# jank324/lynx

Measured on AMD Instinct MI355X. Metric: particle-element-steps/sec (whole node) + achieved HBM GB/s, Segment.track ParticleBeam, higher is better.
Workload: dtype f32

## Files before the change

### lynx_amd/csrc/lynx_device.hpp

```cpp
#pragma once

#include <hip/hip_runtime.h>

#include <type_traits>

#include "lynx_maps.hpp"
#include "lynx_unit_record.hpp"

namespace lynx {

typedef float lynx_f32x4 __attribute__((ext_vector_type(4)));
typedef double lynx_f64x2 __attribute__((ext_vector_type(2)));
template <typename T, bool VEC> struct VecOf { using type = T; static constexpr int width = 1; };
template <> struct VecOf<float, true> { using type = lynx_f32x4; static constexpr int width = 4; };
template <> struct VecOf<double, true> { using type = lynx_f64x2; static constexpr int width = 2; };

struct LatticeDev {
  const lynx_elem* elems;
  const lynx_step* steps;
  const int32_t* elem_step;
  const void* pool;
  int64_t batch;
  int32_t n_elems;
  int32_t n_steps;
};

template <int BYTES>
struct InlinePool {
  uint4 q[BYTES / 16];
};
constexpr int kInlinePoolSmall = 256, kInlinePoolLarge = 1024;
__device__ __forceinline__ LatticeDev inline_pool_view(const LatticeDev& lat) {
  LatticeDev v = lat;
  v.pool = (const void*)__builtin_amdgcn_kernarg_segment_ptr();
  return v;
}

__device__ __forceinline__ bool steps_pair_up(const lynx_step& run, const lynx_step& cav) {
  return run.kind == LYNX_STEP_RUN && cav.kind == LYNX_STEP_CAVITY && !(run.flags & LYNX_STEP_FLAG_OBSERVE);
}

__device__ __forceinline__ int step_descriptor(const LatticeDev& lat, int s, int merge_pairs) {
  const lynx_step st = lat.steps[s];
  int d = (st.flags & 0xffff) | (st.kind << LYNX_DESC_KIND_SHIFT);
  if (merge_pairs && s + 1 < lat.n_steps && steps_pair_up(st, lat.steps[s + 1])) d |= LYNX_DESC_PAIR;
  return d;
}

constexpr double kEntryConditionLimit = 4.0;
template <typename T>
__device__ __forceinline__ bool cavity_entry_inverse(T c44, T c45, T c54, T c55, T (&ci)[4]) {
  const double a = (double)c44 * (double)c55, b = (double)c45 * (double)c54;
  const double det = a - b;
  ci[0] = (T)((double)c55 / det);
  ci[1] = (T)(-(double)c45 / det);
  ci[2] = (T)(-(double)c54 / det);
  ci[3] = (T)((double)c44 / det);
  return !(fabs(det) * kEntryConditionLimit >= fabs(a) + fabs(b)) || det == 0.0;
}

constexpr int kBuildChunk = 64;
constexpr int kTrackThreads = 256;
constexpr int kPartialStride = 36;

template <typename T> __device__ __forceinline__ T shfl_t(T v, int src) { return __shfl(v, src, 64); }

__host__ __device__ inline int build_chunk(int n_elems, int limit = kBuildChunk) {
  return n_elems < limit ? (n_elems > 1 ? n_elems : 1) : limit;
}
__host__ __device__ inline size_t build_scratch_bytes(int chunk, size_t elem_size) {
  size_t b = (size_t)(chunk + (chunk / 2 + 1) + (chunk / 4 + 1) + 2) * 49 * sizeof(double);
  if (elem_size == 4) b += (size_t)chunk * 49 * sizeof(float);
  return (b + 15) / 16 * 16;
}

struct BuildLds {
  size_t steps;
  size_t energies, tail, end;
  size_t total;
};
__host__ __device__ inline BuildLds build_lds_layout(int chunk, size_t n_steps, size_t elem_size, size_t tail_scalars) {
  BuildLds l{};
  l.steps = build_scratch_bytes(chunk, elem_size);
  l.energies = n_steps * LYNX_STEP_STRIDE;
  l.tail = n_steps + 1;
  l.end = tail_scalars;
  l.total = l.steps + (l.energies + l.tail + l.end) * elem_size;
  return l;
// ... 906 lines not shown
}

template <typename T>
__device__ __forceinline__ void build_to_table(const LatticeDev& lat, const T* __restrict__ energy_in,
                                               T* __restrict__ steps_out, T* __restrict__ energy_out,
                                               int chunk, int merge_pairs) {
  extern __shared__ __attribute__((aligned(16))) unsigned char smem_raw[];
  const BuildLds lds = build_lds_layout(chunk, (size_t)lat.n_steps, sizeof(T), 0);
  T* s_steps = reinterpret_cast<T*>(smem_raw + lds.steps);
  T* s_energy = s_steps + lds.energies;
  const int64_t b = blockIdx.x;
  for (int i = threadIdx.x; i < lat.n_steps * LYNX_STEP_STRIDE; i += blockDim.x) s_steps[i] = T(0);
  __syncthreads();
  build_compose_sample<T>(lat, b, energy_in[b], s_steps, s_energy, smem_raw, chunk);
  table_sinphi<T>(lat, s_steps);
  if (merge_pairs) {
    for (int s = 1; s < lat.n_steps; ++s) {
      if (!steps_pair_up(lat.steps[s - 1], lat.steps[s])) continue;
      T* run = s_steps + (s - 1) * LYNX_STEP_STRIDE;
      T* cav = s_steps + s * LYNX_STEP_STRIDE;
      T v = T(0);
      if (threadIdx.x < 49) {
        const int i = threadIdx.x / 7, j = threadIdx.x - i * 7;
        double acc = (double)cav[i * 7] * (double)run[j];
#pragma unroll
        for (int k = 1; k < 7; ++k) acc = fma((double)cav[i * 7 + k], (double)run[k * 7 + j], acc);
        v = (T)acc;
      }
      T ci[4] = {T(0), T(0), T(0), T(0)};
      bool ill = false;
      if (threadIdx.x == 49) ill = cavity_entry_inverse<T>(cav[4 * 7 + 4], cav[4 * 7 + 5], cav[5 * 7 + 4], cav[5 * 7 + 5], ci);
      __syncthreads();
      if (threadIdx.x < 49) cav[threadIdx.x] = v;
      if (threadIdx.x == 49) {
#pragma unroll
        for (int q = 0; q < 4; ++q) cav[LYNX_ENTRY_OFFSET + q] = ci[q];
        cav[LYNX_FLAGS_OFFSET] = ill ? T(1) : T(0);
      }
      if (threadIdx.x >= 64 && threadIdx.x < 78) run[threadIdx.x - 64] = run[28 + (threadIdx.x - 64)];
      __syncthreads();
    }
  }
  for (int s = threadIdx.x; s < lat.n_steps; s += blockDim.x) {
    const bool ill = s_steps[s * LYNX_STEP_STRIDE + LYNX_FLAGS_OFFSET] != T(0);
    s_steps[s * LYNX_STEP_STRIDE + LYNX_FLAGS_OFFSET] = (T)(step_descriptor(lat, s, merge_pairs) | (ill ? LYNX_DESC_ILL : 0));
  }
  if (lat.n_steps > 0 && threadIdx.x == 0)
    s_steps[(lat.n_steps - 1) * LYNX_STEP_STRIDE + LYNX_ENERGY_OFFSET] = s_energy[lat.n_steps];
  __syncthreads();
  T* dst = steps_out + b * (int64_t)lat.n_steps * LYNX_STEP_STRIDE;
  for (int i = threadIdx.x; i < lat.n_steps * LYNX_STEP_STRIDE; i += blockDim.x) dst[i] = s_steps[i];
  if (energy_out && threadIdx.x == 0) energy_out[b] = s_energy[lat.n_steps];
}

template <typename T>
__global__ __launch_bounds__(256) void k_build(LatticeDev lat, const T* __restrict__ energy_in,
                                                T* __restrict__ steps_out, T* __restrict__ energy_out,
                                                int chunk, int merge_pairs) {
  build_to_table<T>(lat, energy_in, steps_out, energy_out, chunk, merge_pairs);
}

template <typename T, int BYTES>
__global__ __launch_bounds__(256) void k_build_inline(InlinePool<BYTES> , LatticeDev lat,
                                                       const T* __restrict__ energy_in, T* __restrict__ steps_out,
                                                       T* __restrict__ energy_out, int chunk, int merge_pairs) {
  build_to_table<T>(inline_pool_view(lat), energy_in, steps_out, energy_out, chunk, merge_pairs);
}


struct TrackArgs {
  int64_t n_particles;
  int32_t chunks;
  int32_t tiles_per_wg;
  int32_t store;
  int32_t lds_scratch_bytes;
  int64_t in_stride;
  int32_t merged_pairs;
  int32_t n_observers;
  uint32_t tail_seq;
  int32_t tail_wg;
  unsigned int* tail_flag;
  int32_t stash_offset;
  int32_t reversed;
};

__device__ __forceinline__ void announce_tail(const TrackArgs& a) {
  if (a.tail_flag && blockIdx.x == (unsigned)a.tail_wg && threadIdx.x == 0)
    __hip_atomic_store(a.tail_flag, a.tail_seq, __ATOMIC_RELAXED, __HIP_MEMORY_SCOPE_SYSTEM);
}

__device__ __forceinline__ float uniform_value(float v) {
  return __int_as_float(__builtin_amdgcn_readfirstlane(__float_as_int(v)));
}
__device__ __forceinline__ double uniform_value(double v) { return v; }
__device__ __forceinline__ float wave_first(float v) { return uniform_value(v); }
__device__ __forceinline__ double wave_first(double v) {
  const long long bits = __double_as_longlong(v);
  const int lo = __builtin_amdgcn_readfirstlane((int)(bits & 0xffffffffll));
  const int hi = __builtin_amdgcn_readfirstlane((int)(bits >> 32));
  return __longlong_as_double(((long long)hi << 32) | (unsigned int)lo);
}

__device__ __forceinline__ double moment_slot_moved(const double* row, const double* c0, int j) {
  if (j == 6 || j >= 28) return row[j];
  const double n = row[35];
  if (j < 6) return row[j] + n * (row[28 + j] - c0[j]);
  int k = j - 7, i = 0, len = 6;
  while (k >= len) { k -= len; --len; ++i; }
  const int jj = i + k;
  const double ei = row[28 + i] - c0[i], ej = row[28 + jj] - c0[jj];
  return row[j] + ei * row[jj] + row[i] * ej + n * ei * ej;
}

template <bool FULL> struct MomentSet {
  static constexpr int N = FULL ? 21 : 8;
  __host__ __device__ static constexpr int row(int k) { return FULL ? tri_row(k) : (k < 6 ? k : (k == 6 ? 0 : 2)); }
  __host__ __device__ static constexpr int col(int k) { return FULL ? tri_col(k) : (k < 6 ? k : (k == 6 ? 1 : 3)); }
  __host__ __device__ static constexpr int slot(int k) { return 7 + tri_index(row(k), col(k)); }
  __host__ __device__ static constexpr int tri_index(int i, int j) { return i * 6 - (i * (i - 1)) / 2 + (j - i); }
  __host__ __device__ static constexpr int tri_row(int k) {
    int i = 0, len = 6;
    while (k >= len) { k -= len; --len; ++i; }
    return i;
  }
  __host__ __device__ static constexpr int tri_col(int k) {
    int i = 0, len = 6;
    while (k >= len) { k -= len; --len; ++i; }
    return i + k;
  }
};

template <typename T, bool FULL> struct MomentAcc {
  using Set = MomentSet<FULL>;
  double d[6], dd[Set::N], one, cnt;
  __device__ __forceinline__ void clear() {
#pragma unroll
    for (int i = 0; i < 6; ++i) d[i] = 0.0;
#pragma unroll
    for (int i = 0; i < Set::N; ++i) dd[i] = 0.0;
    one = 0.0;
    cnt = 0.0;
  }
  template <int K> __device__ __forceinline__ void products(const double (&e)[6]) {
    if constexpr (K < Set::N) {
      constexpr int r = Set::row(K), c = Set::col(K);
      dd[K] = fma(e[r], e[c], dd[K]);
      products<K + 1>(e);
    }
  }
  __device__ __forceinline__ void add(const T (&z)[7], const T (&shift)[6]) {
    double e[6];
#pragma unroll
    for (int i = 0; i < 6; ++i) {
      e[i] = (double)z[i] - (double)shift[i];
      d[i] += e[i];
    }
    one += (double)z[6];
    cnt += 1.0;
    products<0>(e);
  }
};

typedef float lynx_f32x4u __attribute__((ext_vector_type(4), aligned(4)));
typedef float lynx_f32x3u __attribute__((ext_vector_type(3), aligned(4)));
typedef double lynx_f64x2u __attribute__((ext_vector_type(2), aligned(8)));
typedef unsigned int lynx_u32x4 __attribute__((ext_vector_type(4)));
// ... 104 lines not shown
#pragma unroll
    for (int k = 0; k < Set::N; ++k) f_dd[k] = 0.f;
    f_one = 0.f;
  }
  __device__ __forceinline__ void init() {
    if (MOM == 1 || MOM == 2) acc.clear();
    if (MOM == 3) clear_f();
  }
  __device__ __forceinline__ void begin_iteration() {
    if (MOM == 2) clear_f();
  }
  template <int K> __device__ __forceinline__ void products(const float (&e)[6]) {
    if constexpr (K < Set::N) {
      constexpr int r = Set::row(K), c = Set::col(K);
      f_dd[K] = fmaf(e[r], e[c], f_dd[K]);
      products<K + 1>(e);
    }
  }
  __device__ __forceinline__ void add(const T (&z)[7], const T (&shift)[6]) {
    if (MOM == 1) acc.add(z, shift);
    if (MOM == 2 || MOM == 3) {
      float e[6];
#pragma unroll
      for (int k = 0; k < 6; ++k) {
        e[k] = (float)(z[k] - shift[k]);
        f_d[k] += e[k];
      }
      f_one += (float)z[6];
      products<0>(e);
      if (MOM == 2) acc.cnt += 1.0;
      else f_cnt += 1.f;
    }
  }
  __device__ __forceinline__ void end_iteration() {
    if (MOM == 2) {
#pragma unroll
      for (int k = 0; k < 6; ++k) acc.d[k] += (double)f_d[k];
#pragma unroll
      for (int k = 0; k < Set::N; ++k) acc.dd[k] += (double)f_dd[k];
      acc.one += (double)f_one;
    }
  }
  template <typename R> __device__ __forceinline__ void park(R* slab, int lane) const {
    if (MOM == 3) {
#pragma unroll
      for (int i = 0; i < 6; ++i) slab[i * 65 + lane] = (R)f_d[i];
      slab[6 * 65 + lane] = (R)f_one;
#pragma unroll
      for (int i = 0; i < Set::N; ++i) slab[(7 + i) * 65 + lane] = (R)f_dd[i];
      slab[(7 + Set::N) * 65 + lane] = (R)f_cnt;
    } else {
#pragma unroll
      for (int i = 0; i < 6; ++i) slab[i * 65 + lane] = (R)acc.d[i];
      slab[6 * 65 + lane] = (R)acc.one;
#pragma unroll
      for (int i = 0; i < Set::N; ++i) slab[(7 + i) * 65 + lane] = (R)acc.dd[i];
      slab[(7 + Set::N) * 65 + lane] = (R)acc.cnt;
    }
  }
  template <int K> __device__ static __forceinline__ int slot_scan(int r, int sl) {
    if constexpr (K < Set::N) {
      constexpr int slot = Set::slot(K);
      return slot_scan<K + 1>(r, r == 7 + K ? slot : sl);
    } else {
      return sl;
    }
  }
  __device__ static __forceinline__ int slot_of_row(int r) {
    if (r < 7) return r;
    if (r == 7 + Set::N) return 35;
    return slot_scan<0>(r, 0);
  }
};

template <typename T, int MOM, bool FULL>
__device__ __forceinline__ void workgroup_moment_record(const LaneSums<T, MOM, FULL>& sums, const T (&shift)[6],
                                                        unsigned char* s_scratch, double* __restrict__ out) {
  const int tid = threadIdx.x;
  const int wave = tid >> 6, lane = tid & 63;
  {
    using R = typename MomScratch<MOM>::type;
    using Sums = LaneSums<T, MOM, FULL>;
    constexpr int kRows = Sums::kRows;
    __syncthreads();
    R* slab = reinterpret_cast<R*>(s_scratch) + wave * (kRows * 65);
    sums.park(slab, lane);
    __syncthreads();
    double tot = 0.0;
    if (lane < kRows) {
      const R* row = slab + lane * 65;
#pragma unroll 8
      for (int k = 0; k < 64; ++k) tot += (double)row[k];
    }
    __syncthreads();
    double* s_red = reinterpret_cast<double*>(s_scratch);
    if (lane < kPartialStride) s_red[wave * kPartialStride + lane] = 0.0;
    __syncthreads();
    if (lane < kRows) s_red[wave * kPartialStride + Sums::slot_of_row(lane)] = tot;
    if (lane == 0) {
#pragma unroll
      for (int k = 0; k < 6; ++k) s_red[wave * kPartialStride + 28 + k] = (double)shift[k];
      s_red[wave * kPartialStride + 34] = FULL ? 1.0 : 0.0;
    }
    __syncthreads();
    if (tid < kPartialStride) {
      double v;
      if (tid >= 28 && tid < 35) {
        v = s_red[tid];
      } else {
        v = 0.0;
#pragma unroll
        for (int w = 0; w < kTrackThreads / 64; ++w) v += moment_slot_moved(s_red + w * kPartialStride, s_red + 28, tid);
      }
      out[tid] = v;
    }
  }
}

template <typename T, int UNROLL, bool SCALAR_TABLE>
__device__ __forceinline__ void apply_program_lane(const LatticeDev& lat, int S, const T* g_steps, const T* s_steps,
                                                   T (&z)[UNROLL][7],
                                                   double* s_obs = nullptr ,
                                                   const bool (*live)[UNROLL] = nullptr,
                                                   float* stash = nullptr ) {
  constexpr bool kMapInRegs = sizeof(T) == 4;
  constexpr bool kPairs = kMapInRegs && UNROLL % 2 == 0;
  lynx_f32x2 zp[kPairs ? UNROLL / 2 : 1][7];
  if constexpr (kPairs) {
#pragma unroll
    for (int u = 0; u < UNROLL; u += 2)
#pragma unroll
      for (int c = 0; c < 7; ++c) {
        zp[u / 2][c].x = (float)z[u][c];
        zp[u / 2][c].y = (float)z[u + 1][c];
      }
  }
  int n_obs = 0;
  for (int sidx = 0; sidx < S; ++sidx) {
    bool merged = false;
    const T* table = SCALAR_TABLE ? g_steps : s_steps;
    int desc = (int)uniform_value(table[sidx * LYNX_STEP_STRIDE + LYNX_FLAGS_OFFSET]);
    if (s_obs && (desc & LYNX_STEP_FLAG_OBSERVE)) {
#pragma unroll
      for (int u = 0; u < UNROLL; ++u) {
        double x, y;
        if constexpr (kPairs) {
          x = (u & 1) ? (double)zp[u / 2][0].y : (double)zp[u / 2][0].x;
          y = (u & 1) ? (double)zp[u / 2][2].y : (double)zp[u / 2][2].x;
        } else {
          x = (double)z[u][0];
          y = (double)z[u][2];
        }
        if (!live || (*live)[u]) {
          s_obs[(2 * n_obs + 0) * 256] += x;
          s_obs[(2 * n_obs + 1) * 256] += y;
        }
      }
      ++n_obs;
    }
    if constexpr (kPairs && SCALAR_TABLE && UNROLL == 2) {
      if (desc & LYNX_DESC_PAIR) {
        merged = true;
        ++sidx;
        desc = (int)uniform_value(table[sidx * LYNX_STEP_STRIDE + LYNX_FLAGS_OFFSET]);
      }
    }
    const int skind = (desc >> LYNX_DESC_KIND_SHIFT) & 3, sflags = desc & 0xffff;
    if constexpr (kMapInRegs) {
      T m[LYNX_STEP_SCALARS];
      if (SCALAR_TABLE) {
        const T* tab = g_steps + sidx * LYNX_STEP_STRIDE;
#pragma unroll
        for (int q = 0; q < LYNX_STEP_SCALARS; ++q) m[q] = uniform_value(tab[q]);
      } else {
        const T* tab = s_steps + sidx * LYNX_STEP_STRIDE;
#pragma unroll
        for (int q = 0; q < LYNX_STEP_SCALARS; ++q) m[q] = uniform_value(tab[q]);
      }
      if constexpr (kPairs) {
        const bool rows_form = __builtin_expect(merged && (desc & LYNX_DESC_ILL), 0);
        const int entry = !merged ? kEntryOwn : (rows_form ? kEntryStash : kEntryInverse);
#pragma unroll
        for (int h = 0; h < UNROLL / 2; ++h) {
          if (rows_form) {
            lynx_f32x2 s_in = zp[h][0] * uniform_value(g_steps[(sidx - 1) * LYNX_STEP_STRIDE]);
            lynx_f32x2 d_in = zp[h][0] * uniform_value(g_steps[(sidx - 1) * LYNX_STEP_STRIDE + 7]);
#pragma unroll
            for (int j = 1; j < 7; ++j) {
              s_in = pk_fma(zp[h][j], uniform_value(g_steps[(sidx - 1) * LYNX_STEP_STRIDE + j]), s_in);
              d_in = pk_fma(zp[h][j], uniform_value(g_steps[(sidx - 1) * LYNX_STEP_STRIDE + 7 + j]), d_in);
            }
            *reinterpret_cast<lynx_f32x4*>(stash) = lynx_f32x4{s_in.x, s_in.y, d_in.x, d_in.y};
          }
          apply_step_pair(m, skind, sflags, zp[h], entry, lynx_f32x2{0.f, 0.f}, lynx_f32x2{0.f, 0.f}, stash);
        }
      } else {
#pragma unroll
        for (int u = 0; u < UNROLL; ++u) apply_step<T>(m, skind, sflags, z[u]);
      }
    } else {
      const T* tab = s_steps + sidx * LYNX_STEP_STRIDE;
#pragma unroll
      for (int u = 0; u < UNROLL; ++u) apply_step<T>(tab, skind, sflags, z[u]);
    }
  }
  if constexpr (kPairs) {
#pragma unroll
    for (int u = 0; u < UNROLL; u += 2)
#pragma unroll
      for (int c = 0; c < 7; ++c) {
        z[u][c] = (T)zp[u / 2][c].x;
        z[u + 1][c] = (T)zp[u / 2][c].y;
      }
  }
}

template <typename T, int MOM, bool FULL, int UNROLL, bool XPOSE> constexpr int track_waves_per_simd() {
  if (XPOSE) return 3;
  if (sizeof(T) == 4 && UNROLL == 2 && !FULL && (MOM == 0 || MOM == 3)) return 5;
  return 1;
}

struct TrackLds {
  size_t steps, observers, total, stash, stash_bytes;
};
template <typename T>
__host__ __device__ constexpr TrackLds track_lds_layout(size_t scratch_bytes, size_t S, size_t n_observers) {
  TrackLds l{};
  l.steps = scratch_bytes;
  l.observers = (scratch_bytes + (S * (LYNX_STEP_STRIDE + 1) + 1) * sizeof(T) + 7) / 8 * 8;
  l.total = l.observers + 2 * n_observers * 256 * sizeof(double);
  l.stash = (l.total + 15) / 16 * 16;
  l.stash_bytes = (size_t)kTrackThreads * 4 * sizeof(float);
  return l;
}

template <int UNROLL, bool XPOSE>
struct TileGeometry {
  static constexpr int64_t kTile = (int64_t)kTrackThreads * UNROLL;
  static constexpr int64_t kWaveSpan = 64 * UNROLL;
  static constexpr int64_t kLaneStep = XPOSE ? 1 : kTrackThreads;
  int wave, lane, chunk, tiles_per_wg;
  int64_t end;
  int64_t lane_first;
  __device__ __forceinline__ TileGeometry(int tid, int wave_, int lane_, int chunk_, int tiles_per_wg_, int64_t end_)
      : wave(wave_), lane(lane_), chunk(chunk_), tiles_per_wg(tiles_per_wg_), end(end_),
        lane_first(XPOSE ? (int64_t)wave_ * kWaveSpan + (int64_t)lane_ * UNROLL : (int64_t)tid) {}
  __device__ __forceinline__ int64_t tile_of(int it) const { return (int64_t)chunk * tiles_per_wg + it; }
  __device__ __forceinline__ int64_t wave_base(int64_t tile) const { return tile * kTile + (int64_t)wave * kWaveSpan; }
  __device__ __forceinline__ bool wave_whole(int64_t tile) const { return wave_base(tile) + kWaveSpan <= end; }
  __device__ __forceinline__ int64_t first_of(int64_t tile) const { return tile * kTile + lane_first; }
  __device__ __forceinline__ bool past_end(int64_t tile) const { return XPOSE ? (wave_base(tile) >= end) : (first_of(tile) >= end); }
};

template <typename T, int UNROLL>
__device__ __forceinline__ void wave_tile_fetch_if_whole(const TileGeometry<UNROLL, true> g, const T* src, int64_t tile,
                                                         lynx_u32x4 (&v)[7]) {
  if (g.wave_whole(tile)) wave_tile_fetch(src + g.wave_base(tile) * 7, g.lane, v);
}

template <typename T, int N> __device__ __forceinline__ void apply_single_map(const T (&m0)[N], const T* s_steps, T (&z)[7]) {
  if constexpr (sizeof(T) == 4) apply_step<T>(m0, LYNX_STEP_RUN, 0, z);
  else apply_step<T>(s_steps, LYNX_STEP_RUN, 0, z);
}

template <typename T, int MOM, bool FULL, int UNROLL, bool XPOSE>
__global__ __launch_bounds__(kTrackThreads, (track_waves_per_simd<T, MOM, FULL, UNROLL, XPOSE>())) void k_track_direct(
    LatticeDev lat, TrackArgs a, const T* __restrict__ , const T* p_in, T* p_out,
    T* __restrict__ energy_out, const T* __restrict__ steps_in, double* __restrict__ partials,
    double* __restrict__ obs_partials) {
  static_assert(!XPOSE || (UNROLL * 7 * sizeof(T) == 112), "XPOSE: a lane owns 112 bytes");
  extern __shared__ __attribute__((aligned(16))) unsigned char smem_raw[];
  announce_tail(a);
  const TrackLds lds = track_lds_layout<T>(a.lds_scratch_bytes, lat.n_steps, a.n_observers);
  unsigned char* s_scratch = smem_raw;
  T* s_steps = reinterpret_cast<T*>(smem_raw + lds.steps);
  float* stash = reinterpret_cast<float*>(smem_raw + a.stash_offset) + threadIdx.x * 4;
  double* s_obs = reinterpret_cast<double*>(smem_raw + lds.observers) + threadIdx.x;

  const int tid = threadIdx.x;
  const int wave = tid >> 6, lane = tid & 63;
  const unsigned wg = a.reversed ? gridDim.x - 1u - blockIdx.x : blockIdx.x;
  const int64_t b = wg / a.chunks;
  const int chunk = wg % a.chunks;
  const int64_t end = a.n_particles;
  const int S = lat.n_steps;
  using Geometry = TileGeometry<UNROLL, XPOSE>;
  const Geometry g(tid, wave, lane, chunk, a.tiles_per_wg, end);
  unsigned char* s_wave = s_scratch + wave * kWaveTileBytes;

  const T* src = p_in + b * a.in_stride;
  T* dst = p_out + b * end * 7;
  T zn[XPOSE ? 1 : UNROLL][7];
  lynx_u32x4 vn[XPOSE ? 7 : 1];
  if constexpr (XPOSE) {
    wave_tile_fetch_if_whole(g, src, g.tile_of(0), vn);
  } else {
    const int64_t i0 = g.first_of(g.tile_of(0));
#pragma unroll
    for (int u = 0; u < UNROLL; ++u) {
      const int64_t i = i0 + (int64_t)u * Geometry::kLaneStep;
      load_particle(src + (i < end ? i : (i0 < end ? i0 : 0)) * 7, zn[u]);
    }
  }

  const bool one_run = (S == 1) && (lat.steps[0].kind == LYNX_STEP_RUN) && a.n_observers == 0;
  for (int k = 0; k < 2 * a.n_observers; ++k) s_obs[k * 256] = 0.0;
  constexpr bool kMapInRegs = sizeof(T) == 4;
  const T* g_steps = steps_in + b * (int64_t)S * LYNX_STEP_STRIDE;

  if (S > 0) {
    if (!kMapInRegs) load_steps_sample<T>(g_steps, S, s_steps);
    if (energy_out && chunk == 0 && tid == 0) energy_out[b] = g_steps[(S - 1) * LYNX_STEP_STRIDE + LYNX_ENERGY_OFFSET];
  }

  T m0[kMapInRegs ? 49 : 1];
  if (one_run && kMapInRegs) {
#pragma unroll
    for (int i = 0; i < 49; ++i) m0[i] = uniform_value(g_steps[i]);
  }

  LaneSums<T, MOM, FULL> sums;
  sums.init();
  T shift[6];
#pragma unroll
  for (int i = 0; i < 6; ++i) shift[i] = T(0);

  constexpr bool kLdsResident = XPOSE && sizeof(T) == 8;

  for (int it = 0; it < a.tiles_per_wg; ++it) {
    const int64_t tile = g.tile_of(it);
    const int64_t i0 = g.first_of(tile);
    if (g.past_end(tile)) break;
    if (!kMapInRegs) LYNX_FORGET();
    const bool full = XPOSE && g.wave_whole(tile);
    sums.begin_iteration();

    if constexpr (kLdsResident) {
      T* mine =reinterpret_cast<T*>(s_wave) + lane * (UNROLL * 7);
      if (full) {
        lynx_u32x4* l = reinterpret_cast<lynx_u32x4*>(s_wave);
        wave_fence();
#pragma unroll
        for (int k = 0; k < 7; ++k) l[k * 64 + lane] = vn[k];
        wave_fence();
      }
      if (it + 1 < a.tiles_per_wg) wave_tile_fetch_if_whole(g, src, g.tile_of(it + 1), vn);
#pragma unroll 1
      for (int u = 0; u < UNROLL; ++u) {
        const int64_t i = i0 + u;
        T z[1][7];
        if (full) {
#pragma unroll
          for (int c = 0; c < 7; ++c) z[0][c] = mine[u * 7 + c];
        } else {
          load_particle(src + (i < end ? i : end - 1) * 7, z[0]);
        }
        if (one_run) {
          apply_single_map(m0, s_steps, z[0]);
        } else {
          const bool alive[1] = {i < end};
          apply_program_lane<T, 1, false>(lat, S, g_steps, s_steps, z, a.n_observers ? s_obs : nullptr, &alive);
        }
        if (MOM && it == 0 && u == 0) {
#pragma unroll
          for (int k = 0; k < 6; ++k) shift[k] = wave_first(z[0][k]);
        }
        if (i < end) {
          if (MOM) sums.add(z[0], shift);
          if (a.store) {
            if (full) {
#pragma unroll
              for (int c = 0; c < 7; ++c) mine[u * 7 + c] = z[0][c];
            } else {
              store_particle(dst + i * 7, z[0]);
            }
          }
        }
      }
      if (a.store && full) {
        lynx_u32x4 vo[7];
        const lynx_u32x4* l = reinterpret_cast<const lynx_u32x4*>(s_wave);
        wave_fence();
#pragma unroll
        for (int k = 0; k < 7; ++k) vo[k] = l[k * 64 + lane];
        wave_tile_store(dst + g.wave_base(tile) * 7, lane, vo);
      }
    } else {
      T z[UNROLL][7];
      if constexpr (XPOSE) {
        if (full) {
          wave_tile_to_particles<T, UNROLL>(vn, s_wave, lane, z);
        } else {
#pragma unroll
          for (int u = 0; u < UNROLL; ++u) load_particle(src + (i0 + u < end ? i0 + u : end - 1) * 7, z[u]);
        }
        if (it + 1 < a.tiles_per_wg) wave_tile_fetch_if_whole(g, src, g.tile_of(it + 1), vn);
      } else {
#pragma unroll
        for (int u = 0; u < UNROLL; ++u)
#pragma unroll
          for (int c = 0; c < 7; ++c) z[u][c] = zn[u][c];
        if (it + 1 < a.tiles_per_wg) {
          const int64_t j0 = g.first_of(g.tile_of(it + 1));
#pragma unroll
          for (int u = 0; u < UNROLL; ++u) {
            const int64_t j = j0 + (int64_t)u * Geometry::kLaneStep;
            load_particle(src + (j < end ? j : i0) * 7, zn[u]);
          }
        }
      }
      if (!one_run) {
        bool alive[UNROLL];
#pragma unroll
        for (int u = 0; u < UNROLL; ++u) alive[u] = i0 + (int64_t)u * Geometry::kLaneStep < end;
        apply_program_lane<T, UNROLL, kMapInRegs>(lat, S, g_steps, s_steps, z,
                                                  a.n_observers ? s_obs : nullptr, &alive, stash);
      }
#pragma unroll
      for (int u = 0; u < UNROLL; ++u) {
        const int64_t i = i0 + (int64_t)u * Geometry::kLaneStep;
        if (one_run) apply_single_map(m0, s_steps, z[u]);
        if (MOM && it == 0 && u == 0) {
#pragma unroll
          for (int k = 0; k < 6; ++k) shift[k] = wave_first(z[0][k]);
        }
        if (i < end) {
          if (a.store && !(XPOSE && full)) store_particle(dst + i * 7, z[u]);
          if (MOM) sums.add(z[u], shift);
        }
      }
      if constexpr (XPOSE) {
        if (a.store && full) {
          lynx_u32x4 vo[7];
          wave_tile_from_particles<T, UNROLL>(z, s_wave, lane, vo);
          wave_tile_store(dst + g.wave_base(tile) * 7, lane, vo);
        }
      }
    }
    sums.end_iteration();
  }

  if (a.n_observers) {
    __syncthreads();
    if (tid < 2 * a.n_observers) {
      const double* row = s_obs - threadIdx.x + tid * 256;
      double tot = 0.0;
      for (int k = 0; k < 256; ++k) tot += row[k];
      obs_partials[((int64_t)b * a.chunks + chunk) * (2 * LYNX_MAX_OBSERVERS) + tid] = tot;
    }
  }

  if (MOM) workgroup_moment_record<T, MOM, FULL>(sums, shift, s_scratch, partials + ((int64_t)b * a.chunks + chunk) * kPartialStride);
}

constexpr int kReduceStage = 70;
template <int THREADS, int STAGE> constexpr size_t reduce_lds_bytes() {
  return (size_t)(STAGE + THREADS / kPartialStride + 1) * kPartialStride * sizeof(double);
}

__device__ __forceinline__ void write_moment_record(const double* s, double* dst, int tid) {
  const double n = s[35];
  if (tid < 6) {
    dst[tid] = s[28 + tid] + s[tid] / n;
  } else if (tid == 6) {
    dst[6] = s[6] / n;
  } else if (tid < 28) {
    int k = tid - 7, i = 0, row = 6;
    while (k >= row) { k -= row; --row; ++i; }
    const int j = i + k;
    const bool have = (s[34] != 0.0 || i == j || (i == 0 && j == 1) || (i == 2 && j == 3)) &&
                      __builtin_isfinite(s[i]) && __builtin_isfinite(s[j]);
    dst[tid] = have ? (s[tid] - s[i] * s[j] / n) / n : __longlong_as_double(0x7ff8000000000000ll);
  } else if (tid < 34) {
    dst[tid] = 0.0;
  } else if (tid == 34) {
    dst[34] = s[34];
  } else if (tid == 35) {
    dst[35] = n;
  }
}

struct ReduceLds {
  double *rows, *set, *s;
};
template <int THREADS, int STAGE>
// ... 692 lines not shown
```

### lynx_amd/csrc/lynx_hip.hip

```cpp
#include <hip/hip_runtime.h>
#include <hip/hip_ext.h>
#include <rccl/rccl.h>

#include <algorithm>
#include <array>
#include <cstdio>
#include <cstdlib>
#include <cstring>
#include <map>
#include <mutex>
#include <string>
#include <type_traits>
#include <unordered_map>
#include <vector>

#include "lynx_device.hpp"
#include "lynx_grad.hpp"
#include "lynx_units.hpp"
#include "lynx_grad_units.hpp"
#include "lynx_trace.hpp"
#include "lynx_trace_grad.hpp"
#include "lynx_trace_jvp.hpp"
#include "lynx_moment_loss.hpp"

using namespace lynx;

struct Knobs {
  int xpose = -1;
  int unroll = -1;
  int mom = -1;
  int min_tiles_per_wg = -1;
  int async_build = -1;
  int side_reduce = -1;
  int build_host_wait = -1;
  int gather_overlap = -1;
  int lanes_build_min_batch = 256;
  int piece = 8;
  int pair_levels_fused = 1;
  int merge_steps = 1;
  int reduce_ticket = 1;
  int one_round = -1;
  int track_units = 1;
  int unit_pairs = 1;
  int bwd_units = 1;
  int bwd_merge = 1;
  int bwd_pairs = 1;
  int build_in_tail = 1;
  int small_inline = -1;
  int bwd_reuse_table = 1;
  int host_visible_records = 1;
  int alternate_order = 1;
  int inline_pool = 1;
};

static void load_knobs(Knobs* k) {
  *k = Knobs();
  const struct { const char* name; int* value; } table[] = {
      {"LYNX_XPOSE", &k->xpose}, {"LYNX_UNROLL", &k->unroll}, {"LYNX_MOM", &k->mom},
      {"LYNX_MIN_TILES_PER_WG", &k->min_tiles_per_wg}, {"LYNX_ASYNC_BUILD", &k->async_build},
      {"LYNX_SIDE_REDUCE", &k->side_reduce}, {"LYNX_BUILD_HOST_WAIT", &k->build_host_wait},
      {"LYNX_GATHER_OVERLAP", &k->gather_overlap}, {"LYNX_LANES_BUILD_MIN_BATCH", &k->lanes_build_min_batch},
      {"LYNX_PIECE", &k->piece}, {"LYNX_PAIR_LEVELS_FUSED", &k->pair_levels_fused},
      {"LYNX_MERGE_STEPS", &k->merge_steps},
      {"LYNX_REDUCE_TICKET", &k->reduce_ticket}, {"LYNX_TRACK_UNITS", &k->track_units}, {"LYNX_ONE_ROUND", &k->one_round}, {"LYNX_UNIT_PAIRS", &k->unit_pairs}, {"LYNX_BWD_UNITS", &k->bwd_units},
      {"LYNX_BWD_MERGE", &k->bwd_merge}, {"LYNX_BWD_PAIRS", &k->bwd_pairs}, {"LYNX_BUILD_IN_TAIL", &k->build_in_tail},
      {"LYNX_SMALL_INLINE", &k->small_inline}, {"LYNX_INLINE_POOL", &k->inline_pool}, {"LYNX_ALTERNATE_ORDER", &k->alternate_order}, {"LYNX_HOST_VISIBLE_RECORDS", &k->host_visible_records}, {"LYNX_BWD_REUSE_TABLE", &k->bwd_reuse_table}};
  for (const auto& t : table) {
    const char* v = getenv(t.name);
    if (v && *v) *t.value = atoi(v);
  }
}
static inline int knob(int value, int dflt) { return value >= 0 ? value : dflt; }

struct Scratch {
  void* buf = nullptr;
  size_t bytes = 0;
};

struct lynx_ctx {
  Knobs knobs;
  int device = 0;
  hipStream_t stream = nullptr;
  hipStream_t s_build = nullptr;
  static constexpr int kTableSlots = 3;
  hipEvent_t ev_built[kTableSlots] = {};
  struct BuildOrder {
    hipEvent_t ev_streamed_own[kTableSlots] = {}, ev_mark = nullptr;
    hipEvent_t ev_streamed[kTableSlots] = {};
    bool streamed_valid[kTableSlots] = {};
    bool main_dirty = false;
    const void* main_wrote = nullptr;
    const void* slot_wrote[kTableSlots] = {};

    void main_wrote_build_input() { main_dirty = true; }
    hipEvent_t stop_event(int slot) const { return ev_streamed_own[slot]; }
    void streamed(int slot, bool async, hipEvent_t stop, const void* energy_out) {
      if (slot >= 0) {
        ev_streamed[slot] = stop;
        streamed_valid[slot] = async && stop != nullptr;
        if (!async) main_dirty = true;
        slot_wrote[slot] = energy_out;
      }
      if (energy_out) main_wrote = energy_out;
    }
    hipError_t read_until_here(int slot, hipStream_t main) {
      const hipError_t e = hipEventRecord(ev_streamed_own[slot], main);
      if (e != hipSuccess) return e;
      ev_streamed[slot] = ev_streamed_own[slot];
      streamed_valid[slot] = true;
      return hipSuccess;
    }
    hipError_t order_build(hipStream_t bs, hipStream_t main, int slot, const void* energy, unsigned int* tail_flag,
                           uint32_t tail_value) {
      hipError_t e = hipSuccess;
      if (streamed_valid[slot] && (e = hipStreamWaitEvent(bs, ev_streamed[slot], 0)) != hipSuccess) return e;
      if (tail_flag && (e = hipStreamWaitValue32(bs, tail_flag, tail_value, hipStreamWaitValueGte, 0xffffffffu)) != hipSuccess)
        return e;
      if (main_dirty || (main_wrote && main_wrote == energy)) {
        if ((e = hipEventRecord(ev_mark, main)) != hipSuccess || (e = hipStreamWaitEvent(bs, ev_mark, 0)) != hipSuccess) return e;
        main_dirty = false;
        main_wrote = nullptr;
        for (const void*& w : slot_wrote) w = nullptr;
      } else {
        for (int i = 0; i < kTableSlots; ++i)
          if (i != slot && slot_wrote[i] == energy && energy && streamed_valid[i] &&
              (e = hipStreamWaitEvent(bs, ev_streamed[i], 0)) != hipSuccess)
            return e;
      }
      return hipSuccess;
    }
    void forget_stop_events() {
      for (bool& v : streamed_valid) v = false;
    }
  } order;
  unsigned seq = 0;
  bool main_idle = true;
  bool plain_events = false;
  unsigned long_calls = 0;
  struct FwdTable {
    const lynx_lattice* lat = nullptr;
    uint64_t version = 0;
    const void* energy = nullptr;
    int slot = -1;
    int merged = 0;
    bool units = false;
    size_t energy_bytes = 0;
    unsigned seq = 0;
    bool valid = false;
    void written(const void* dst, size_t bytes) {
// ... 1134 lines not shown
  }
  const int chunk = fit_build_chunk<T>(build_shape<T>(ctx, lat, underneath, true), lat, 0);
  const size_t lds = build_lds_layout(chunk, (size_t)lat->n_steps, sizeof(T), 0).total;
  const auto launch = [&](const auto&... pool) -> int {
    const auto kernel = build_kernel<T>(pool...);
    if constexpr (sizeof...(pool) == 0)
      if (const int stale = sync_pool(ctx, lat)) return stale;
    if (const int refused = allow_lds(ctx, kernel, lds)) return refused;
    hipLaunchKernelGGL(kernel, dim3((unsigned)lat->batch), dim3(256), lds, stream, pool..., dev_view(lat), (const T*)d_energy_in,
                       (T*)d_steps_out, (T*)d_energy_out, chunk, merge_pairs);
    HIP_TRY(ctx, hipGetLastError());
    return LYNX_OK;
  };
  if (const int rc = with_pool_form<T>(lat, lat->prog_pool && ctx->knobs.inline_pool, launch)) return rc;
  if constexpr (sizeof(T) == 4)
    if (d_units) return launch_pack_units(ctx, lat, merge_pairs, stream, d_steps_out, d_units, d_extras);
  return LYNX_OK;
}

int lynx_build_compose(lynx_ctx* ctx, lynx_lattice* lat, const void* d_energy_in, void* d_steps_out,
                       void* d_energy_out) {
  LYNX_MAIN_ENTRY(ctx);
  if (!lat || !d_energy_in || !d_steps_out) return fail(ctx, LYNX_ERR_INVALID, "null argument");
  if (lat->batch > 0x7fffffffLL) return fail(ctx, LYNX_ERR_INVALID, "batch too large");
  const size_t es = dtype_size(lat->dtype);
  LYNX_MAIN_WRITES(ctx, kFeedsBuild, {{d_steps_out, (size_t)lat->batch * lat->n_steps * LYNX_STEP_STRIDE * es},
                                      {d_energy_out, (size_t)lat->batch * es}});
  return with_dtype(lat->dtype, [&](auto zero) {
    return launch_build<decltype(zero)>(ctx, lat, ctx->stream, d_energy_in, d_steps_out, d_energy_out);
  });
}


struct TrackPlan {
  hipEvent_t done = nullptr;
  bool full_cov;
  int unroll;
  int mom_mode;
  bool xpose;
  TrackArgs a;
  size_t lds;
  unsigned grid;
};

template <typename T>
static TrackPlan plan_track(lynx_ctx* ctx, const lynx_lattice* lat, int64_t B, int64_t N, int32_t S, bool moments,
                            bool full_cov) {
  TrackPlan p;
  p.full_cov = full_cov;
  constexpr int P = 16 / (int)sizeof(T);
  const int64_t cus = compute_units(ctx);
  const Knobs& kn = ctx->knobs;
  const int64_t target = 512 * cus;
  p.mom_mode = knob(kn.mom, sizeof(T) == 4 ? 2 : 1);
  if (sizeof(T) == 8 || p.mom_mode < 2 || p.mom_mode > 3) p.mom_mode = sizeof(T) == 4 ? 2 : 1;
  p.a.n_particles = N;
  p.a.store = 0;
  p.a.tail_flag = nullptr;
  p.a.tail_seq = 0;
  p.a.tail_wg = 0;
  p.a.stash_offset = 0;
  p.a.reversed = 0;
  const bool single_map = S == 1 && lat && lat->h_steps[0].kind == LYNX_STEP_RUN &&
                          !(lat->h_steps[0].flags & LYNX_STEP_FLAG_OBSERVE);
  p.xpose = knob(kn.xpose, ((sizeof(T) == 8 || (single_map && !full_cov)) && N >= 8 * 64 * P) ? 1 : 0) != 0;
  int u = knob(kn.unroll, p.xpose ? P : (sizeof(T) == 4 ? (S > 1 ? 2 : 4) : 1));
  if (u != 1 && u != 2 && u != 4) u = 2;
  if (sizeof(T) == 8 && u > 2) u = 2;
  while (u > 1 && B * ((N + 256 * u - 1) / (256 * u)) < 4 * cus) u >>= 1;
  if (u != P) p.xpose = false;
  p.unroll = u;
  const int64_t tile = 256 * (int64_t)u;
  const int64_t ntiles = (N + tile - 1) / tile;
  int64_t min_tpw = std::max(1, knob(kn.min_tiles_per_wg, S > 1 ? 16 : 2));
  while (min_tpw > 1 && B * ((ntiles + min_tpw - 1) / min_tpw) < 4 * cus) --min_tpw;
  int64_t chunks = std::max<int64_t>(1, std::min<int64_t>((ntiles + min_tpw - 1) / min_tpw, (target + B - 1) / B));
  {
    const int64_t one_round = 3 * cus;
    const int cap = knob(kn.one_round, (S <= 1 && B * chunks > one_round && B * chunks <= 4 * one_round) ? 3 : 0);
    if (cap > 0) chunks = std::max<int64_t>(1, std::min<int64_t>(chunks, cap * cus / B));
  }
  int64_t tpw = (ntiles + chunks - 1) / chunks;
  chunks = (ntiles + tpw - 1) / tpw;
  p.a.chunks = (int32_t)chunks;
  p.a.tiles_per_wg = (int32_t)tpw;
  if (p.mom_mode == 2 && kn.mom < 0 && tpw * u <= 32) p.mom_mode = 3;
  if (p.mom_mode == 3 && tpw * u > 64) p.mom_mode = 2;
  size_t scratch = 4 * kPartialStride * sizeof(double);
  if (moments)
    scratch = std::max<size_t>(scratch, (size_t)(full_cov ? kMomSlabScalars : kMomSlabScalarsCompact) * (p.mom_mode >= 2 ? 4 : 8));
  if (p.xpose) scratch = std::max<size_t>(scratch, (size_t)(kTrackThreads / 64) * kWaveTileBytes);
  scratch = (scratch + 15) / 16 * 16;
  p.a.lds_scratch_bytes = (int32_t)scratch;
  p.a.n_observers = lat ? lat->n_observers : 0;
  p.lds = track_lds_layout<T>(scratch, (size_t)S, (size_t)p.a.n_observers).total;
  p.grid = (unsigned)(B * chunks);
  return p;
}

template <typename K, typename... Args>
static int launch_streaming(lynx_ctx* ctx, const TrackPlan& p, K kernel, size_t lds, const Args&... args) {
  int rc = allow_lds(ctx, kernel, lds);
  if (rc) return rc;
  hipEvent_t e0 = nullptr, e1 = p.done;
  if (ctx->profiling) {
    HIP_TRY(ctx, hipEventCreateWithFlags(&e0, timing_event_flags(ctx)));
    HIP_TRY(ctx, hipEventCreateWithFlags(&e1, timing_event_flags(ctx)));
  }
  hipExtLaunchKernelGGL(kernel, dim3(p.grid), dim3(kTrackThreads), (std::uint32_t)lds, ctx->stream, e0, e1, 0u, args...);
  HIP_TRY(ctx, hipGetLastError());
  if (ctx->profiling) ctx->prof_events.emplace_back(e0, e1);
  ctx->last_stream_stop = e1;
  return LYNX_OK;
}

struct DirectLaunch {
  lynx_ctx* ctx;
  const TrackPlan& p;
  const LatticeDev& lv;
  const void *d_energy_in, *d_p_in;
  void *d_p_out, *d_energy_out;
  const void* d_steps;
  double *d_partials, *d_obs;
};

template <typename T, int MOM, bool FULL, int UNROLL, bool XPOSE>
static int launch_direct_inst(const DirectLaunch& l) {
  return launch_streaming(l.ctx, l.p, k_track_direct<T, MOM, FULL, UNROLL, XPOSE>, l.p.lds, l.lv, l.p.a, (const T*)l.d_energy_in,
                          (const T*)l.d_p_in, (T*)l.d_p_out, (T*)l.d_energy_out, (const T*)l.d_steps, l.d_partials, l.d_obs);
}

template <typename T, int MOM, bool FULL, int U>
static int launch_direct_mu(const DirectLaunch& l) {
  if constexpr (U * 7 * sizeof(T) == 112) {
    if (l.p.xpose) return launch_direct_inst<T, MOM, FULL, U, true>(l);
  }
  return launch_direct_inst<T, MOM, FULL, U, false>(l);
}

template <typename T, int MOM, bool FULL>
static int launch_direct_m(const DirectLaunch& l) {
  switch (l.p.unroll) {
    case 1: return launch_direct_mu<T, MOM, FULL, 1>(l);
    case 2: return launch_direct_mu<T, MOM, FULL, 2>(l);
    default:
      if constexpr (sizeof(T) == 4) return launch_direct_mu<T, MOM, FULL, 4>(l);
      else return fail(l.ctx, LYNX_ERR_INVALID, "float64: at most 2 particles per lane");
  }
}

template <typename T>
static int launch_direct(const DirectLaunch& l, bool moments) {
  const int mom = moments ? l.p.mom_mode : 0;
  if (mom == 0) return launch_direct_m<T, 0, false>(l);
  if constexpr (sizeof(T) == 4) {
    if (mom == 3) return l.p.full_cov ? launch_direct_m<T, 3, true>(l) : launch_direct_m<T, 3, false>(l);
    return l.p.full_cov ? launch_direct_m<T, 2, true>(l) : launch_direct_m<T, 2, false>(l);
  } else {
    return l.p.full_cov ? launch_direct_m<T, 1, true>(l) : launch_direct_m<T, 1, false>(l);
  }
}


static int proposed_class(const lynx_lattice* lat, int32_t first, int32_t last) {
  int rank = 1;
  for (int32_t e = first; e < last; ++e) {
// ... 2181 lines not shown
```

Before: 13970 billion.

## Add tapered chunk plan and wave-local moment reduction in tracking kernel

Adds a launch plan in which the last chunks of each sample handle a single tile each, with chunk-major workgroup ordering, so the tail of the grid finishes more evenly. This mode is gated behind a new LYNX_TAPER knob that defaults to off. The moment record reduction is also rewritten to run inside each wave, using 16-row passes with shuffles and wave fences in place of several workgroup barriers. Each wave's record is kept inside its own slab, which cuts synchronisation in the epilogue but depends on the slab size assertions holding.

```diff
diff --git a/lynx_amd/csrc/lynx_device.hpp b/lynx_amd/csrc/lynx_device.hpp
--- a/lynx_amd/csrc/lynx_device.hpp
+++ b/lynx_amd/csrc/lynx_device.hpp
@@ -4,6 +4,7 @@
 
 #include <type_traits>
 
+#include "lynx_launch_plan.hpp"
 #include "lynx_maps.hpp"
 #include "lynx_unit_record.hpp"
 
@@ -1076,6 +1077,9 @@
   unsigned int* tail_flag;
   int32_t stash_offset;
   int32_t reversed;
+  TilePlan tiles;
+  int32_t chunk_major;
+  int32_t batch;
 };
 
 __device__ __forceinline__ void announce_tail(const TrackArgs& a) {
@@ -1346,35 +1350,49 @@
     using R = typename MomScratch<MOM>::type;
     using Sums = LaneSums<T, MOM, FULL>;
     constexpr int kRows = Sums::kRows;
+    constexpr int kSlabBytes = kRows * 65 * (int)sizeof(R);
+    static_assert(kRows <= 32, "two passes of 16 rows");
+    static_assert(kPartialStride * 8 + 7 <= kSlabBytes, "a wave's record, on whole float64 cells, lies inside its own slab");
     __syncthreads();
     R* slab = reinterpret_cast<R*>(s_scratch) + wave * (kRows * 65);
     sums.park(slab, lane);
-    __syncthreads();
-    double tot = 0.0;
-    if (lane < kRows) {
-      const R* row = slab + lane * 65;
-#pragma unroll 8
-      for (int k = 0; k < 64; ++k) tot += (double)row[k];
-    }
-    __syncthreads();
-    double* s_red = reinterpret_cast<double*>(s_scratch);
-    if (lane < kPartialStride) s_red[wave * kPartialStride + lane] = 0.0;
-    __syncthreads();
-    if (lane < kRows) s_red[wave * kPartialStride + Sums::slot_of_row(lane)] = tot;
+    wave_fence();
+    const int r = lane & 15, q = lane >> 4;
+    double tot[2] = {0.0, 0.0};
+#pragma unroll
+    for (int pass = 0; pass < (kRows > 16 ? 2 : 1); ++pass) {
+      if (pass * 16 + r < kRows) {
+        const R* cells = slab + (pass * 16 + r) * 65 + q * 16;
+#pragma unroll
+        for (int k = 0; k < 16; ++k) tot[pass] += (double)cells[k];
+      }
+      tot[pass] += __shfl_down(tot[pass], 16);
+      tot[pass] += __shfl_down(tot[pass], 32);
+    }
+    double* s_rec = reinterpret_cast<double*>(s_scratch) + (wave * kSlabBytes + 7) / 8;
+    wave_fence();
+    if (lane < kPartialStride) s_rec[lane] = 0.0;
+    wave_fence();
+    if (lane < 16) {
+      s_rec[Sums::slot_of_row(lane)] = tot[0];
+      if (kRows > 16 && 16 + lane < kRows) s_rec[Sums::slot_of_row(16 + lane)] = tot[1];
+    }
     if (lane == 0) {
 #pragma unroll
-      for (int k = 0; k < 6; ++k) s_red[wave * kPartialStride + 28 + k] = (double)shift[k];
-      s_red[wave * kPartialStride + 34] = FULL ? 1.0 : 0.0;
+      for (int k = 0; k < 6; ++k) s_rec[28 + k] = (double)shift[k];
+      s_rec[34] = FULL ? 1.0 : 0.0;
     }
     __syncthreads();
     if (tid < kPartialStride) {
+      const double* s_red = reinterpret_cast<const double*>(s_scratch);
+      const auto rec = [&](int w) { return s_red + (w * kSlabBytes + 7) / 8; };
       double v;
       if (tid >= 28 && tid < 35) {
-        v = s_red[tid];
+        v = rec(0)[tid];
       } else {
         v = 0.0;
 #pragma unroll
-        for (int w = 0; w < kTrackThreads / 64; ++w) v += moment_slot_moved(s_red + w * kPartialStride, s_red + 28, tid);
+        for (int w = 0; w < kTrackThreads / 64; ++w) v += moment_slot_moved(rec(w), rec(0) + 28, tid);
       }
       out[tid] = v;
     }
@@ -1504,13 +1522,14 @@
   static constexpr int64_t kTile = (int64_t)kTrackThreads * UNROLL;
   static constexpr int64_t kWaveSpan = 64 * UNROLL;
   static constexpr int64_t kLaneStep = XPOSE ? 1 : kTrackThreads;
-  int wave, lane, chunk, tiles_per_wg;
+  int wave, lane;
+  TileSpan tiles;
   int64_t end;
   int64_t lane_first;
-  __device__ __forceinline__ TileGeometry(int tid, int wave_, int lane_, int chunk_, int tiles_per_wg_, int64_t end_)
-      : wave(wave_), lane(lane_), chunk(chunk_), tiles_per_wg(tiles_per_wg_), end(end_),
+  __device__ __forceinline__ TileGeometry(int tid, int wave_, int lane_, TileSpan tiles_, int64_t end_)
+      : wave(wave_), lane(lane_), tiles(tiles_), end(end_),
         lane_first(XPOSE ? (int64_t)wave_ * kWaveSpan + (int64_t)lane_ * UNROLL : (int64_t)tid) {}
-  __device__ __forceinline__ int64_t tile_of(int it) const { return (int64_t)chunk * tiles_per_wg + it; }
+  __device__ __forceinline__ int64_t tile_of(int it) const { return (int64_t)tiles.first + it; }
   __device__ __forceinline__ int64_t wave_base(int64_t tile) const { return tile * kTile + (int64_t)wave * kWaveSpan; }
   __device__ __forceinline__ bool wave_whole(int64_t tile) const { return wave_base(tile) + kWaveSpan <= end; }
   __device__ __forceinline__ int64_t first_of(int64_t tile) const { return tile * kTile + lane_first; }
@@ -1544,13 +1563,19 @@
 
   const int tid = threadIdx.x;
   const int wave = tid >> 6, lane = tid & 63;
-  const unsigned wg = a.reversed ? gridDim.x - 1u - blockIdx.x : blockIdx.x;
-  const int64_t b = wg / a.chunks;
-  const int chunk = wg % a.chunks;
+  ChunkOfSample at;
+  if (a.chunk_major) {
+    at = chunk_major_position(a.tiles, blockIdx.x, (uint32_t)a.batch, a.reversed != 0);
+  } else {
+    const unsigned wg = a.reversed ? gridDim.x - 1u - blockIdx.x : blockIdx.x;
+    at = ChunkOfSample{(int32_t)(wg / a.chunks), (int32_t)(wg % a.chunks)};
+  }
+  const int64_t b = at.sample;
+  const int chunk = at.chunk;
   const int64_t end = a.n_particles;
   const int S = lat.n_steps;
   using Geometry = TileGeometry<UNROLL, XPOSE>;
-  const Geometry g(tid, wave, lane, chunk, a.tiles_per_wg, end);
+  const Geometry g(tid, wave, lane, chunk_tiles(a.tiles, chunk), end);
   unsigned char* s_wave = s_scratch + wave * kWaveTileBytes;
 
   const T* src = p_in + b * a.in_stride;
@@ -1592,7 +1617,7 @@
 
   constexpr bool kLdsResident = XPOSE && sizeof(T) == 8;
 
-  for (int it = 0; it < a.tiles_per_wg; ++it) {
+  for (int it = 0; it < g.tiles.count; ++it) {
     const int64_t tile = g.tile_of(it);
     const int64_t i0 = g.first_of(tile);
     if (g.past_end(tile)) break;
@@ -1609,7 +1634,7 @@
         for (int k = 0; k < 7; ++k) l[k * 64 + lane] = vn[k];
         wave_fence();
       }
-      if (it + 1 < a.tiles_per_wg) wave_tile_fetch_if_whole(g, src, g.tile_of(it + 1), vn);
+      if (it + 1 < g.tiles.count) wave_tile_fetch_if_whole(g, src, g.tile_of(it + 1), vn);
 #pragma unroll 1
       for (int u = 0; u < UNROLL; ++u) {
         const int64_t i = i0 + u;
@@ -1659,13 +1684,13 @@
 #pragma unroll
           for (int u = 0; u < UNROLL; ++u) load_particle(src + (i0 + u < end ? i0 + u : end - 1) * 7, z[u]);
         }
-        if (it + 1 < a.tiles_per_wg) wave_tile_fetch_if_whole(g, src, g.tile_of(it + 1), vn);
+        if (it + 1 < g.tiles.count) wave_tile_fetch_if_whole(g, src, g.tile_of(it + 1), vn);
       } else {
 #pragma unroll
         for (int u = 0; u < UNROLL; ++u)
 #pragma unroll
           for (int c = 0; c < 7; ++c) z[u][c] = zn[u][c];
-        if (it + 1 < a.tiles_per_wg) {
+        if (it + 1 < g.tiles.count) {
           const int64_t j0 = g.first_of(g.tile_of(it + 1));
 #pragma unroll
           for (int u = 0; u < UNROLL; ++u) {
diff --git a/lynx_amd/csrc/lynx_hip.hip b/lynx_amd/csrc/lynx_hip.hip
--- a/lynx_amd/csrc/lynx_hip.hip
+++ b/lynx_amd/csrc/lynx_hip.hip
@@ -49,6 +49,7 @@
   int small_inline = -1;
   int bwd_reuse_table = 1;
   int host_visible_records = 1;
+  int taper = 0;
   int alternate_order = 1;
   int inline_pool = 1;
 };
@@ -64,7 +65,7 @@
       {"LYNX_MERGE_STEPS", &k->merge_steps},
       {"LYNX_REDUCE_TICKET", &k->reduce_ticket}, {"LYNX_TRACK_UNITS", &k->track_units}, {"LYNX_ONE_ROUND", &k->one_round}, {"LYNX_UNIT_PAIRS", &k->unit_pairs}, {"LYNX_BWD_UNITS", &k->bwd_units},
       {"LYNX_BWD_MERGE", &k->bwd_merge}, {"LYNX_BWD_PAIRS", &k->bwd_pairs}, {"LYNX_BUILD_IN_TAIL", &k->build_in_tail},
-      {"LYNX_SMALL_INLINE", &k->small_inline}, {"LYNX_INLINE_POOL", &k->inline_pool}, {"LYNX_ALTERNATE_ORDER", &k->alternate_order}, {"LYNX_HOST_VISIBLE_RECORDS", &k->host_visible_records}, {"LYNX_BWD_REUSE_TABLE", &k->bwd_reuse_table}};
+      {"LYNX_SMALL_INLINE", &k->small_inline}, {"LYNX_INLINE_POOL", &k->inline_pool}, {"LYNX_ALTERNATE_ORDER", &k->alternate_order}, {"LYNX_TAPER", &k->taper}, {"LYNX_HOST_VISIBLE_RECORDS", &k->host_visible_records}, {"LYNX_BWD_REUSE_TABLE", &k->bwd_reuse_table}};
   for (const auto& t : table) {
     const char* v = getenv(t.name);
     if (v && *v) *t.value = atoi(v);
@@ -1365,6 +1366,21 @@
   }
   int64_t tpw = (ntiles + chunks - 1) / chunks;
   chunks = (ntiles + tpw - 1) / tpw;
+  p.a.tiles = uniform_plan((int32_t)chunks, (int32_t)tpw);
+  p.a.chunk_major = 0;
+  p.a.batch = (int32_t)B;
+  {
+    int64_t taper = 0;
+    if (single_map && ntiles <= 0x7fffffffLL && kn.taper > 0) {
+      taper = std::min<int64_t>(kn.taper, ntiles);
+      if (kn.min_tiles_per_wg > 0) tpw = kn.min_tiles_per_wg;
+    }
+    if (taper > 0) {
+      chunks = tapered_chunks((int32_t)ntiles, (int32_t)tpw, (int32_t)taper);
+      p.a.tiles = tapered_plan((int32_t)ntiles, (int32_t)chunks, (int32_t)taper);
+      p.a.chunk_major = 1;
+    }
+  }
   p.a.chunks = (int32_t)chunks;
   p.a.tiles_per_wg = (int32_t)tpw;
   if (p.mom_mode == 2 && kn.mom < 0 && tpw * u <= 32) p.mom_mode = 3;
diff --git a/lynx_amd/csrc/lynx_launch_plan.hpp b/lynx_amd/csrc/lynx_launch_plan.hpp
--- /dev/null
+++ b/lynx_amd/csrc/lynx_launch_plan.hpp
@@ -0,0 +1,58 @@
+#pragma once
+#include <cstdint>
+
+#if defined(__HIPCC__) || defined(__CUDACC__)
+#define LYNX_PLAN_HD __host__ __device__ __forceinline__
+#else
+#define LYNX_PLAN_HD inline
+#endif
+
+namespace lynx {
+
+struct TilePlan {
+  int32_t body;
+  int32_t base;
+  int32_t rem;
+};
+struct TileSpan {
+  int32_t first, count;
+};
+
+LYNX_PLAN_HD int32_t taper_allowed(int32_t ntiles, int32_t chunks, int32_t taper) {
+  if (taper < 0) taper = 0;
+  if (taper > chunks) taper = chunks;
+  if (taper == chunks && ntiles > chunks) taper = chunks - 1;
+  return taper;
+}
+
+LYNX_PLAN_HD TilePlan tapered_plan(int32_t ntiles, int32_t chunks, int32_t taper) {
+  const int32_t t = taper_allowed(ntiles, chunks, taper);
+  TilePlan p;
+  p.body = chunks - t;
+  p.base = p.body ? (ntiles - t) / p.body : 0;
+  p.rem = p.body ? (ntiles - t) % p.body : 0;
+  return p;
+}
+
+LYNX_PLAN_HD TilePlan uniform_plan(int32_t chunks, int32_t tiles_per_wg) { return TilePlan{chunks, tiles_per_wg, 0}; }
+
+LYNX_PLAN_HD int32_t tapered_chunks(int32_t ntiles, int32_t tiles_per_wg, int32_t taper) {
+  const int32_t t = taper < ntiles ? (taper > 0 ? taper : 0) : ntiles;
+  return t + (ntiles - t + tiles_per_wg - 1) / tiles_per_wg;
+}
+
+LYNX_PLAN_HD TileSpan chunk_tiles(const TilePlan& p, int32_t chunk) {
+  if (chunk >= p.body) return TileSpan{p.body * p.base + p.rem + (chunk - p.body), 1};
+  return TileSpan{chunk * p.base + (chunk < p.rem ? chunk : p.rem), p.base + (chunk < p.rem ? 1 : 0)};
+}
+
+struct ChunkOfSample {
+  int32_t sample, chunk;
+};
+LYNX_PLAN_HD ChunkOfSample chunk_major_position(const TilePlan& p, uint32_t wg, uint32_t batch, bool reversed) {
+  const int32_t pos = (int32_t)(wg / batch), s = (int32_t)(wg % batch);
+  if (!reversed) return ChunkOfSample{s, pos};
+  return ChunkOfSample{(int32_t)batch - 1 - s, pos < p.body ? p.body - 1 - pos : pos};
+}
+
+}
```

Result: no change. 14100 billion, median of 6 (+0.9%).
